# livesense-inc/fanlin-rs

Measured on AMD Instinct MI355X. Metric: images/sec whole-node (1080p→300×200 resize+encode); p50 per-image ms, higher is better.
Workload: dtype u8 (exact, as f16 subnormals) x the reference's f32 weights as three f16 terms -> f32 sums (vertical, v_mfma_f32_16x16x32_f16); 24-bit fixed-point intermediate (2^-14 steps, three i8 planes) x 24-bit fixed-point weights (2^-24 steps, three i8 digits), eight of the nine digit products -> exact i32 (h

## Files before the change

### fanlin-rs_amd/csrc/fl_jpeg.hip

```cpp
#include <hip/hip_runtime.h>
#include <stdint.h>

#include "fl_jpeg.h"
#include "fl_jpeg_tables.h"
#include "fl_pixel.h"
#include "fl_types.h"

namespace fl {

namespace {


constexpr int32_t F_0_298 = 2446, F_0_390 = 3196, F_0_541 = 4433, F_0_765 = 6270, F_0_899 = 7373, F_1_175 = 9633, F_1_501 = 12299,
                  F_1_847 = 15137, F_1_961 = 16069, F_2_053 = 16819, F_2_562 = 20995, F_3_072 = 25172;

struct Mat8 { int32_t a[8][8]; };

constexpr void fdct_linear(const int32_t in[8], int32_t out[8])
{
    int32_t t0 = in[0] + in[7], t1 = in[1] + in[6], t2 = in[2] + in[5], t3 = in[3] + in[4];
    const int32_t t10 = t0 + t3, t11 = t1 + t2;
    int32_t t12 = t0 - t3, t13 = t1 - t2;
    t0 = in[0] - in[7]; t1 = in[1] - in[6]; t2 = in[2] - in[5]; t3 = in[3] - in[4];
    out[0] = t10 + t11;
    out[4] = t10 - t11;
    int32_t z1 = (t12 + t13) * F_0_541;
    out[2] = z1 + t12 * F_0_765;
    out[6] = z1 - t13 * F_1_847;
    t12 = t0 + t2;
    t13 = t1 + t3;
    z1 = (t12 + t13) * F_1_175;
    t12 = t12 * (-F_0_390) + z1;
    t13 = t13 * (-F_1_961) + z1;
    z1 = (t0 + t3) * (-F_0_899);
    out[1] = t0 * F_1_501 + z1 + t12;
    out[7] = t3 * F_0_298 + z1 + t13;
    z1 = (t1 + t2) * (-F_2_562);
    out[3] = t1 * F_3_072 + z1 + t13;
    out[5] = t2 * F_2_053 + z1 + t12;
}

constexpr Mat8 make_fdct_matrix()
{
    Mat8 m{};
    for (int j = 0; j < 8; ++j) {
        int32_t e[8] = {0, 0, 0, 0, 0, 0, 0, 0}, o[8] = {0, 0, 0, 0, 0, 0, 0, 0};
        e[j] = 1;
        fdct_linear(e, o);
        for (int k = 0; k < 8; ++k) m.a[k][j] = o[k];
    }
    return m;
}

__constant__ Mat8 kFdct = make_fdct_matrix();

constexpr bool fdct_matrix_fits_i16()
{
    const Mat8 m = make_fdct_matrix();
    for (int k = 0; k < 8; ++k)
        for (int j = 0; j < 8; ++j)
            if (m.a[k][j] > 32767 || m.a[k][j] < -32768) return false;
    return true;
}
static_assert(fdct_matrix_fits_i16(), "the passes use v_dot2_i32_i16: matrix entries must be 16-bit");

typedef short i16x2 __attribute__((ext_vector_type(2)));
__device__ __forceinline__ i16x2 as_i16x2(uint32_t v) { return __builtin_bit_cast(i16x2, v); }
__device__ __forceinline__ uint32_t pack_i16(int32_t lo, int32_t hi) { return ((uint32_t)lo & 0xffffu) | ((uint32_t)hi << 16); }
__device__ __forceinline__ int32_t dot8_i16(const uint32_t m[4], const uint4 v)
{
    int32_t p = __builtin_amdgcn_sdot2(as_i16x2(m[0]), as_i16x2(v.x), 0, false);
    p = __builtin_amdgcn_sdot2(as_i16x2(m[1]), as_i16x2(v.y), p, false);
    p = __builtin_amdgcn_sdot2(as_i16x2(m[2]), as_i16x2(v.z), p, false);
    return __builtin_amdgcn_sdot2(as_i16x2(m[3]), as_i16x2(v.w), p, false);
}

struct NaturalOrder { uint8_t n[64]; };
constexpr NaturalOrder make_natural()
{
    NaturalOrder t{};
    for (int k = 0; k < 64; ++k) t.n[k] = kUnzigzag[k];
    return t;
}
__constant__ NaturalOrder kNatural = make_natural();

struct HuffLut { uint32_t e[256]; };

constexpr HuffLut make_lut(const HuffSpec &s)
{
    HuffLut t{};
    uint32_t code = 0;
    int k = 0;
    for (int l = 1; l <= 16; ++l) {
        for (int i = 0; i < s.len[l - 1]; ++i, ++k) t.e[s.val[k]] = ((uint32_t)l << 16) | code++;
        code <<= 1;
    }
    return t;
}

struct HuffAll { HuffLut ac[2], dc[2]; };
constexpr HuffAll make_all() { return HuffAll{{make_lut(kAcLuma), make_lut(kAcChroma)}, {make_lut(kDcLuma), make_lut(kDcChroma)}}; }
__constant__ HuffAll kHuff = make_all();


template <int N>
__device__ __forceinline__ uint32_t dpp_row_shr(uint32_t v)
{
    return (uint32_t)__builtin_amdgcn_update_dpp(0, (int)v, 0x110 + N, 0xf, 0xf, false);
}

__device__ __forceinline__ uint32_t wave_inclusive_scan(uint32_t v, uint32_t lane)
{
    (void)lane;
    v += dpp_row_shr<1>(v);
    v += dpp_row_shr<2>(v);
    v += dpp_row_shr<4>(v);
    v += dpp_row_shr<8>(v);
    v += (uint32_t)__builtin_amdgcn_update_dpp(0, (int)v, 0x142, 0xa, 0xf, false);
    v += (uint32_t)__builtin_amdgcn_update_dpp(0, (int)v, 0x143, 0xc, 0xf, false);
    return v;
}

__device__ __forceinline__ void wave_lds_sync()
{
    __builtin_amdgcn_fence(__ATOMIC_SEQ_CST, "wavefront");
    __builtin_amdgcn_wave_barrier();
}

constexpr uint32_t kPackThreads = 512;
constexpr uint32_t kPackWaves = kPackThreads / 64;

__device__ __forceinline__ uint32_t wg_exclusive_scan(uint32_t v, uint32_t *s_w, uint32_t *total)
{
    const uint32_t lane = threadIdx.x & 63u, wave = threadIdx.x >> 6;
    const uint32_t inc = wave_inclusive_scan(v, lane);
    __syncthreads();
    if (lane == 63u) s_w[wave] = inc;
    __syncthreads();
    uint32_t base = 0, sum = 0;
#pragma unroll
    for (uint32_t i = 0; i < kPackWaves; ++i) { const uint32_t t = s_w[i]; if (i < wave) base += t; sum += t; }
    *total = sum;
    return base + inc - v;
}

__device__ __forceinline__ uint32_t coef_size(int32_t v)
{
    const uint32_t mag = (uint32_t)(v < 0 ? -v : v);
    return mag ? 32u - (uint32_t)__clz(mag) : 0u;
}


#ifndef FL_JPEG_BPW
#define FL_JPEG_BPW 16
#define FL_JPEG_WPG 2
#define FL_JPEG_PREFETCH 3
#endif
constexpr uint32_t kBlocksPerWave = FL_JPEG_BPW;
constexpr uint32_t kWavesPerWg = FL_JPEG_WPG;
constexpr uint32_t kPrefetch = FL_JPEG_PREFETCH;
static_assert(kBlocksPerWave == 32u || kBlocksPerWave == 16u, "the coding phase's lane mapping");
constexpr uint32_t kJpegThreads = 64u * kWavesPerWg;
constexpr uint32_t kBlocksPerWg = kWavesPerWg * kBlocksPerWave;
constexpr uint32_t kUnitsPerWave = 3u * kBlocksPerWave;

static_assert(63u * (16u + 10u) <= kAcWordsPerUnit * 32u, "a unit's AC code must fit its acbits slot");

struct WaveLds {
    int16_t coef[kUnitsPerWave][64];
    uint64_t nz[kUnitsPerWave];
    __attribute__((aligned(16))) int16_t smp[3][64];
    __attribute__((aligned(16))) int16_t p1[3][64];
};

__device__ __forceinline__ void stage_ac_luts(uint32_t *s_ac)
{
    for (uint32_t i = threadIdx.x; i < 512u; i += kJpegThreads) s_ac[i] = kHuff.ac[i >> 8].e[i & 255u];
    __syncthreads();
}

template <bool kRgba>
__device__ __forceinline__ uint32_t block_pixel(const JpegJob &jb, uint32_t brow, uint32_t bcol, uint32_t r, uint32_t c)
{
    uint32_t px = bcol * 8u + c, py = brow * 8u + r;
    px = px < jb.w ? px : jb.w - 1u;
    py = py < jb.h ? py : jb.h - 1u;
    if constexpr (kRgba) return ((const __attribute__((address_space(1))) uint32_t *)jb.src)[(size_t)py * jb.w + px];
    uint32_t pr, pg, pb, pa;
    load_rgba(jb.src + ((size_t)py * jb.w + px) * jb.c, jb.c, pr, pg, pb, pa);
    return pr | (pg << 8) | (pb << 16);
}

__device__ __forceinline__ void dct_quant_block(const uint32_t (&smp)[3], uint32_t nat, uint32_t r, uint32_t c, const uint32_t (&m1)[4],
                                                const uint32_t (&m2)[4], uint4 k1, const uint32_t (&q)[3], const uint32_t (&magic)[3],
                                                WaveLds &w, int32_t (&qv)[3])
{
#pragma unroll
    for (int k = 0; k < 3; ++k) w.smp[k][nat] = (int16_t)smp[k];
    wave_lds_sync();
#pragma unroll
    for (int k = 0; k < 3; ++k) {
        const int32_t p = dot8_i16(m1, *reinterpret_cast<const uint4 *>(w.smp[k] + r * 8));
        const int32_t v1 = ((p << k1.x) + (int32_t)k1.y) >> 11;
        w.p1[k][c * 8 + r] = (int16_t)v1;
    }
    wave_lds_sync();
#pragma unroll
    for (int k = 0; k < 3; ++k) {
        const int32_t p2 = dot8_i16(m2, *reinterpret_cast<const uint4 *>(w.p1[k] + c * 8));
        const int32_t d = (p2 + (int32_t)k1.z) >> k1.w;
        const int32_t sg = d >> 31;
        const uint32_t an = (uint32_t)((d ^ sg) - sg) >> 3;
        const uint32_t rq = __umulhi(2u * an + q[k], magic[k]);
        qv[k] = ((int32_t)rq ^ sg) - sg;
    }
}

typedef __attribute__((address_space(1))) uint32_t global_u32;
typedef uint32_t u32x4 __attribute__((ext_vector_type(4)));
typedef __attribute__((address_space(1))) u32x4 global_u32x4;
static_assert(sizeof(JpegUnit) == sizeof(u32x4) && kUnitAcWords == 3u, "a unit's record is one 16-byte access");

struct UnitBits {
    uint64_t acc;
    uint32_t pend, total, wi;
    global_u32 *out;
    uint32_t w0, w1, w2;
    __device__ __forceinline__ void word(uint32_t v)
    {
        w0 = wi == 0u ? v : w0;
        w1 = wi == 1u ? v : w1;
        w2 = wi == 2u ? v : w2;
        if (wi >= kUnitAcWords) out[wi] = v;
        ++wi;
    }
    __device__ __forceinline__ void put(uint32_t code, uint32_t len)
    {
        acc = (acc << len) | code;
        pend += len;
        total += len;
        if (pend >= 32u) { pend -= 32u; word((uint32_t)(acc >> pend)); }
    }
};

template <bool kRgba>
__device__ __forceinline__ void transform_blocks(const JpegJob &jb, const uint32_t *__restrict__ arena, uint32_t first, uint32_t count,
                                                 uint32_t lane, WaveLds &w)
{
    const uint32_t nat = kNatural.n[lane], r = nat >> 3, c = nat & 7u;
    uint32_t m1[4], m2[4];
#pragma unroll
    for (int j = 0; j < 4; ++j) {
        m1[j] = pack_i16(kFdct.a[c][2 * j], kFdct.a[c][2 * j + 1]);
        m2[j] = pack_i16(kFdct.a[r][2 * j], kFdct.a[r][2 * j + 1]);
    }
    const uint8_t *qt = reinterpret_cast<const uint8_t *>(arena + jb.tab_off) + 624;
    const uint32_t *mg = reinterpret_cast<const uint32_t *>(qt + 128);
    const uint32_t q[3] = {qt[nat], qt[64 + nat], qt[64 + nat]};
    const uint32_t magic[3] = {mg[nat], mg[64 + nat], mg[64 + nat]};
    const uint4 k1 = {(c == 0u || c == 4u) ? 13u : 0u, c == 0u ? (uint32_t)(-(8 * 128) * 8192) : (c == 4u ? 0u : 1u << 10),
                      (r == 0u || r == 4u) ? 2u : 1u << 14, (r == 0u || r == 4u) ? 2u : 15u};
    uint32_t brow = first / jb.bx, bcol = first - brow * jb.bx;
    uint32_t ahead[kPrefetch];
#pragma unroll
    for (uint32_t j = 0; j < kPrefetch; ++j) {
        ahead[j] = block_pixel<kRgba>(jb, brow, bcol, r, c);
        if (++bcol == jb.bx) { bcol = 0; ++brow; }
    }
    for (uint32_t i = 0; i < count; ++i) {
        const uint32_t rgb = kRgba ? ahead[0] & 0xffffffu : ahead[0];
#pragma unroll
        for (uint32_t j = 0; j + 1u < kPrefetch; ++j) ahead[j] = ahead[j + 1u];
        ahead[kPrefetch - 1u] = block_pixel<kRgba>(jb, brow, bcol, r, c);
        if (++bcol == jb.bx) { bcol = 0; ++brow; }
        uint32_t smp[3];
        jfif_px(rgb, smp[0], smp[1], smp[2]);
        const bool flat = __ballot(rgb != (uint32_t)__builtin_amdgcn_readfirstlane((int)rgb)) == 0ull;
        if (flat) {
            if (lane == 0u) {
#pragma unroll
                for (int k = 0; k < 3; ++k) {
                    const int32_t d = 64 * ((int32_t)smp[k] - 128);
                    const int32_t sg = d >> 31;
                    const uint32_t an = (uint32_t)((d ^ sg) - sg) >> 3;
                    const uint32_t rq = __umulhi(2u * an + q[k], magic[k]);
                    w.coef[i * 3u + k][0] = (int16_t)(((int32_t)rq ^ sg) - sg);
                    w.nz[i * 3u + k] = 0ull;
                }
            }
            continue;
        }
        int32_t qv[3];
        dct_quant_block(smp, nat, r, c, m1, m2, k1, q, magic, w, qv);
#pragma unroll
        for (int k = 0; k < 3; ++k) {
            w.coef[i * 3u + k][lane] = (int16_t)qv[k];
            const uint64_t nz = __ballot(qv[k] != 0) & ~1ull;
            if (lane == 0u) w.nz[i * 3u + k] = nz;
        }
    }
}

__global__ __launch_bounds__(kJpegThreads) void jpeg_dct_quant_kernel(const JpegJob *__restrict__ jobs, const uint32_t *__restrict__ arena,
                                                                      uint32_t job_base)
{
    __shared__ WaveLds s_w[kWavesPerWg];
    __shared__ uint32_t s_ac[512];
    const JpegJob jb = jobs[job_base + blockIdx.y];
    const uint32_t wave = threadIdx.x >> 6, lane = threadIdx.x & 63u;
    const uint32_t nblocks = jb.bx * jb.by;
    if (blockIdx.x * kBlocksPerWg >= nblocks) return;
    stage_ac_luts(s_ac);
    const uint32_t first = blockIdx.x * kBlocksPerWg + wave * kBlocksPerWave;
    if (first >= nblocks) return;
    const uint32_t count = min(kBlocksPerWave, nblocks - first);
    WaveLds &w = s_w[wave];

    if (jb.c == 4u && (reinterpret_cast<uintptr_t>(jb.src) & 3u) == 0u) transform_blocks<true>(jb, arena, first, count, lane, w);
    else transform_blocks<false>(jb, arena, first, count, lane, w);
    wave_lds_sync();

    uint32_t b, u, u_end;
    bool chroma;
    if constexpr (kBlocksPerWave == 32u) {
        b = lane & 31u;
        chroma = lane >= 32u;
        u = b * 3u + (chroma ? 1u : 0u);
        u_end = b * 3u + (chroma ? 3u : 1u);
    } else {
        b = lane & 15u;
        chroma = lane >= 16u;
        u = b * 3u + (lane >> 4);
        u_end = lane >= 48u ? u : u + 1u;
    }
    if (b >= count) return;
    const uint32_t *tab = s_ac + (chroma ? 256u : 0u);
    const uint32_t eob = tab[0], zrl = tab[0xF0];
    for (; u < u_end; ++u) {
        const uint32_t unit = first * 3u + u;
        const int16_t *cf = w.coef[u];
        uint64_t m = w.nz[u];
        UnitBits ub{0ull, 0u, 0u, 0u, (global_u32 *)jb.acbits + (size_t)unit * kAcWordsPerUnit, 0u, 0u, 0u};
        uint32_t prev = 0;
        uint32_t pos = (uint32_t)__builtin_ctzll(m | (1ull << 63));
        int32_t v = cf[pos];
        while (m) {
            const uint32_t cpos = pos;
            const int32_t cv = v;
            m &= m - 1ull;
            pos = (uint32_t)__builtin_ctzll(m | (1ull << 63));
            v = cf[pos];
            uint32_t run = cpos - prev - 1u;
            prev = cpos;
            while (run > 15u) { ub.put(zrl & 0xffffu, zrl >> 16); run -= 16u; }
            const uint32_t mag = (uint32_t)(cv < 0 ? -cv : cv);
            const uint32_t size = 32u - (uint32_t)__clz(mag);
            const uint32_t value = (uint32_t)(cv + (cv >> 31)) & ((1u << size) - 1u);
            const uint32_t e = tab[(run << 4) | size];
            ub.put(((e & 0xffffu) << size) | value, (e >> 16) + size);
        }
        if (prev != 63u) ub.put(eob & 0xffffu, eob >> 16);
        if (ub.pend) ub.word((uint32_t)(ub.acc << (32u - ub.pend)));
        const u32x4 rec = {((uint32_t)(uint16_t)cf[0]) | (ub.total << 16), ub.w0, ub.w1, ub.w2};
        ((global_u32x4 *)jb.units)[unit] = rec;
    }
}


constexpr uint32_t kWinWords = 8192;

__device__ __forceinline__ void win_or(uint32_t *win, uint32_t wbase, uint64_t g, uint32_t val)
{
    const uint64_t W = g >> 5;
    const uint32_t sh = (uint32_t)g & 31u;
    const uint32_t hi = val >> sh, lo = sh ? val << (32u - sh) : 0u;
    if (hi && W >= wbase && W < (uint64_t)wbase + kWinWords) atomicOr(&win[W - wbase], hi);
    if (lo && W + 1 >= wbase && W + 1 < (uint64_t)wbase + kWinWords) atomicOr(&win[W + 1 - wbase], lo);
}

constexpr uint32_t kDcCodes = 12;

__device__ __forceinline__ uint32_t dc_code(const uint32_t *s_dc, uint32_t u, uint32_t meta, uint32_t prev_meta, uint32_t *len)
{
    const int32_t dc = (int16_t)(meta & 0xffffu), prev = (int16_t)(prev_meta & 0xffffu);
    const int32_t diff = dc - prev;
    const uint32_t size = coef_size(diff);
    const uint32_t value = (uint32_t)(diff < 0 ? diff - 1 : diff) & ((1u << size) - 1u);
    const uint32_t e = s_dc[((u % 3u) ? kDcCodes : 0u) + size];
    *len = (e >> 16) + size;
    return (((e & 0xffffu) << size) | value) << (32u - *len);
}

struct PackUnit { u32x4 rec; uint32_t prev; };
__device__ __forceinline__ PackUnit load_pack_unit(const JpegJob &jb, uint32_t u, uint32_t u_end)
{
    const global_u32x4 *recs = (const global_u32x4 *)jb.units;
    const uint32_t uc = min(u, u_end - 1u);
    PackUnit p;
    p.rec = recs[uc];
    p.prev = ((const global_u32 *)(recs + (max(uc, 3u) - 3u)))[0];
    return p;
}
__device__ __forceinline__ PackUnit take_pack_unit(PackUnit p, uint32_t u, uint32_t u_end)
{
    if (u >= u_end) p.rec = u32x4{0u, 0u, 0u, 0u};
    if (u < 3u || u >= u_end) p.prev = 0u;
    return p;
}

#ifndef FL_JPEG_PACK_DEPTH
#define FL_JPEG_PACK_DEPTH 1
#endif
constexpr uint32_t kPackDepth = FL_JPEG_PACK_DEPTH;

__global__ __launch_bounds__(kPackThreads) void jpeg_pack_kernel(const JpegJob *__restrict__ jobs, const uint32_t *__restrict__ arena,
                                                                 uint32_t job_base)
{
    __shared__ uint32_t s_win[kWinWords];
    __shared__ uint32_t s_w[kPackWaves], s_carry, s_lo, s_hi, s_dc[2u * kDcCodes];
    const JpegJob jb = jobs[job_base + blockIdx.x];
    const uint32_t tid = threadIdx.x;
    const uint32_t nunits = jb.bx * jb.by * 3u;
    constexpr uint32_t T = kPackThreads;

    PackUnit ahead[kPackDepth];
#pragma unroll
    for (uint32_t j = 0; j < kPackDepth; ++j) ahead[j] = load_pack_unit(jb, j * T + tid, nunits);
    for (uint32_t i = tid; i < kWinWords; i += T) s_win[i] = 0u;
    if (tid < 2u * kDcCodes) s_dc[tid] = kHuff.dc[tid / kDcCodes].e[tid % kDcCodes];
    if (tid == 0u) s_carry = 0u;
    __syncthreads();
    for (uint32_t base0 = 0; base0 < nunits; base0 += kPackDepth * T) {
#pragma unroll
        for (uint32_t j = 0; j < kPackDepth; ++j) {
            const uint32_t base = base0 + j * T;
            if (base >= nunits) break;
            const uint32_t u = base + tid;
            const PackUnit next = load_pack_unit(jb, u + kPackDepth * T, nunits);
            const PackUnit cur = take_pack_unit(ahead[j], u, nunits);
            ahead[j] = next;
            const uint32_t m = cur.rec.x;
            const uint32_t nw = ((m >> 16) + 31u) >> 5;
            uint32_t len = 0, dl = 0, dcw = 0;
            if (u < nunits) {
                dcw = dc_code(s_dc, u, m, cur.prev, &dl);
                len = dl + (m >> 16);
            }
            uint32_t chunk;
            const uint32_t ex = wg_exclusive_scan(len, s_w, &chunk);
            const uint32_t carry = s_carry;
            if (u < nunits) {
                const uint32_t off = carry + ex;
                ((global_u32 *)jb.unit_off)[u] = off;
                win_or(s_win, 0u, off, dcw);
                win_or(s_win, 0u, (uint64_t)off + dl, cur.rec.y);
                win_or(s_win, 0u, (uint64_t)off + dl + 32u, cur.rec.z);
                win_or(s_win, 0u, (uint64_t)off + dl + 64u, cur.rec.w);
                for (uint32_t w = kUnitAcWords; w < nw; ++w)
                    win_or(s_win, 0u, (uint64_t)off + dl + 32u * w, ((const global_u32 *)jb.acbits)[(size_t)u * kAcWordsPerUnit + w]);
            }
            __syncthreads();
            if (tid == 0u) s_carry = carry + chunk;
            __syncthreads();
        }
    }
    const uint32_t total_bits = s_carry;
    if (tid == 0u) jb.unit_off[nunits] = total_bits;
    __threadfence_block();
    __syncthreads();
    const uint32_t nbytes = (total_bits + 7u) >> 3, limit = jb.dst_cap;
    const uint8_t *hdr = reinterpret_cast<const uint8_t *>(arena + jb.tab_off);
    for (uint32_t i = tid; i < kJpegHeaderBytes; i += T) if (i < limit) jb.dst[i] = hdr[i];

    uint32_t ff_before = 0;
    for (uint32_t wbase = 0; wbase * 32ull < total_bits; wbase += kWinWords) {
        const uint64_t wb = (uint64_t)wbase * 32u, we = wb + (uint64_t)kWinWords * 32u;
        if (wbase != 0u) {
            for (uint32_t i = tid; i < kWinWords; i += T) s_win[i] = 0u;
            if (tid == 0u) {
                uint32_t lo = 0, hi = nunits;
                while (lo < hi) { const uint32_t mid = (lo + hi) >> 1; if (jb.unit_off[mid + 1u] > wb) hi = mid; else lo = mid + 1u; }
                s_lo = lo;
                uint32_t lo2 = lo, hi2 = nunits;
                while (lo2 < hi2) { const uint32_t mid = (lo2 + hi2) >> 1; if (jb.unit_off[mid] >= we) hi2 = mid; else lo2 = mid + 1u; }
                s_hi = lo2;
            }
        } else if (tid == 0u) { s_lo = 0u; s_hi = 0u; }
        __syncthreads();
        const uint32_t u_lo = s_lo, u_hi = s_hi;
        for (uint32_t ub = u_lo; ub < u_hi; ub += T / 2u) {
            const uint32_t u = ub + (tid >> 1), j = tid & 1u;
            if (u < u_hi) {
                const PackUnit p = take_pack_unit(load_pack_unit(jb, u, u_hi), u, u_hi);
                const uint32_t m = p.rec.x, off = jb.unit_off[u];
                uint32_t dl;
                const uint32_t dcw = dc_code(s_dc, u, m, p.prev, &dl);
                if (j == 0u) win_or(s_win, wbase, off, dcw);
                const uint32_t nw = ((m >> 16) + 31u) >> 5;
                win_or(s_win, wbase, (uint64_t)off + dl + 32u * j, j ? p.rec.z : p.rec.y);
                if (j == 0u) win_or(s_win, wbase, (uint64_t)off + dl + 64u, p.rec.w);
                for (uint32_t w = j ? 3u : 4u; w < nw; w += 2u)
                    win_or(s_win, wbase, (uint64_t)off + dl + 32u * w, ((const global_u32 *)jb.acbits)[(size_t)u * kAcWordsPerUnit + w]);
            }
        }
        __syncthreads();
        if (tid == 0u && (total_bits & 7u) && (total_bits >> 5) >= wbase && (total_bits >> 5) < wbase + kWinWords)
            s_win[(total_bits >> 5) - wbase] |= (0xFFu >> (total_bits & 7u)) << (24u - 8u * ((total_bits >> 3) & 3u));
        __syncthreads();
        const uint32_t win_bytes = (uint32_t)min((uint64_t)kWinWords * 4u, (uint64_t)nbytes - (uint64_t)wbase * 4u);
        if (tid == 0u) s_carry = 0u;
        __syncthreads();
        for (uint32_t base = 0; base < win_bytes; base += 4u * T) {
            const uint32_t i = base + tid * 4u;
            const uint32_t word = i < win_bytes ? s_win[i >> 2] : 0u;
            const uint32_t valid = i < win_bytes ? (win_bytes - i < 4u ? win_bytes - i : 4u) : 0u;
            uint32_t ff = 0;
#pragma unroll
            for (uint32_t k = 0; k < 4; ++k) ff += (k < valid && ((word >> (24u - 8u * k)) & 255u) == 255u) ? 1u : 0u;
            uint32_t chunk;
            const uint32_t ex = wg_exclusive_scan(ff, s_w, &chunk);
            const uint32_t carry = s_carry;
            uint64_t o = (uint64_t)kJpegHeaderBytes + (uint64_t)wbase * 4u + i + ff_before + carry + ex;
#pragma unroll
            for (uint32_t k = 0; k < 4; ++k) {
                if (k < valid) {
                    const uint32_t b = (word >> (24u - 8u * k)) & 255u;
                    if (o < limit) jb.dst[o] = (uint8_t)b;
                    ++o;
                    if (b == 255u) { if (o < limit) jb.dst[o] = 0u; ++o; }
                }
            }
            __syncthreads();
            if (tid == 0u) s_carry = carry + chunk;
            __syncthreads();
        }
        ff_before += s_carry;
        __syncthreads();
    }
    if (tid == 0u) {
        const uint64_t end = (uint64_t)kJpegHeaderBytes + nbytes + ff_before;
        if (end + 2u <= limit) {
            jb.dst[end] = 0xFF; jb.dst[end + 1u] = 0xD9;
            jb.result[1] = (uint32_t)(end + 2u);
        } else {
            jb.result[1] = 0u;
            atomicOr(&jb.result[0], FL_JPEG_RESULT_OVERFLOW);
        }
    }
}

}

hipError_t launch_jpeg_encode(const JpegJob *jobs, const uint32_t *arena, uint32_t job_base, uint32_t njobs, uint32_t max_blocks,
                              hipStream_t st)
{
    if (!njobs || !max_blocks) return hipSuccess;
    hipLaunchKernelGGL(jpeg_dct_quant_kernel, dim3((max_blocks + kBlocksPerWg - 1) / kBlocksPerWg, njobs), dim3(kJpegThreads), 0, st, jobs, arena, job_base);
    FL_LAUNCH_CHECK();
    hipLaunchKernelGGL(jpeg_pack_kernel, dim3(njobs), dim3(kPackThreads), 0, st, jobs, arena, job_base);
    FL_LAUNCH_CHECK();
    return hipSuccess;
}

}
```

Before: 558,700.

## Fold DCT rounding into dot seeds, use 32-bit pixel offsets, ring-buffer prefetch

Moves the pass-1 scale and bias into the DCT matrix and into the sdot2 accumulator seed, and folds the quantiser's shift and doubling into precomputed constants, which removes several ALU ops per coefficient. Adds a 32-bit offset path (v_mad_u32_u24) for pixel addressing when the image dimensions allow it, avoiding 64-bit address arithmetic. Replaces the shifting prefetch array with an indexed ring unrolled over kPrefetch and adds a sched_barrier. It also batches the lane-0 nz stores. The changed rounding constants must stay bit-exact, and the template instantiations double, which grows code size.

```diff
diff --git a/fanlin-rs_amd/csrc/fl_jpeg.hip b/fanlin-rs_amd/csrc/fl_jpeg.hip
--- a/fanlin-rs_amd/csrc/fl_jpeg.hip
+++ b/fanlin-rs_amd/csrc/fl_jpeg.hip
@@ -67,9 +67,9 @@
 typedef short i16x2 __attribute__((ext_vector_type(2)));
 __device__ __forceinline__ i16x2 as_i16x2(uint32_t v) { return __builtin_bit_cast(i16x2, v); }
 __device__ __forceinline__ uint32_t pack_i16(int32_t lo, int32_t hi) { return ((uint32_t)lo & 0xffffu) | ((uint32_t)hi << 16); }
-__device__ __forceinline__ int32_t dot8_i16(const uint32_t m[4], const uint4 v)
-{
-    int32_t p = __builtin_amdgcn_sdot2(as_i16x2(m[0]), as_i16x2(v.x), 0, false);
+__device__ __forceinline__ int32_t dot8_i16(const uint32_t m[4], const uint4 v, int32_t seed)
+{
+    int32_t p = __builtin_amdgcn_sdot2(as_i16x2(m[0]), as_i16x2(v.x), seed, false);
     p = __builtin_amdgcn_sdot2(as_i16x2(m[1]), as_i16x2(v.y), p, false);
     p = __builtin_amdgcn_sdot2(as_i16x2(m[2]), as_i16x2(v.z), p, false);
     return __builtin_amdgcn_sdot2(as_i16x2(m[3]), as_i16x2(v.w), p, false);
@@ -179,20 +179,39 @@
     __syncthreads();
 }
 
-template <bool kRgba>
+template <bool kRgba, bool kOff32>
 __device__ __forceinline__ uint32_t block_pixel(const JpegJob &jb, uint32_t brow, uint32_t bcol, uint32_t r, uint32_t c)
 {
     uint32_t px = bcol * 8u + c, py = brow * 8u + r;
     px = px < jb.w ? px : jb.w - 1u;
     py = py < jb.h ? py : jb.h - 1u;
+    if constexpr (kRgba && kOff32) {
+        uint32_t idx;
+        asm("v_mad_u32_u24 %0, %1, %2, %3" : "=v"(idx) : "v"(py), "s"(jb.w), "v"(px));
+        const uint32_t off = idx << 2;
+        return *(const __attribute__((address_space(1))) uint32_t *)((const __attribute__((address_space(1))) uint8_t *)jb.src + off);
+    }
     if constexpr (kRgba) return ((const __attribute__((address_space(1))) uint32_t *)jb.src)[(size_t)py * jb.w + px];
     uint32_t pr, pg, pb, pa;
-    load_rgba(jb.src + ((size_t)py * jb.w + px) * jb.c, jb.c, pr, pg, pb, pa);
+    if constexpr (kOff32) load_rgba(jb.src + ((py & 0xffffffu) * ((jb.w * jb.c) & 0xffffffu) + (px & 0xffffffu) * (jb.c & 0xffffffu)), jb.c, pr, pg, pb, pa);
+    else load_rgba(jb.src + ((size_t)py * jb.w + px) * jb.c, jb.c, pr, pg, pb, pa);
     return pr | (pg << 8) | (pb << 16);
 }
 
+__device__ __forceinline__ bool jpeg_offsets_fit_32bits(const JpegJob &jb)
+{
+    return (jb.w | jb.h) < 65536u && (uint64_t)(jb.w * jb.h) * jb.c <= (1ull << 32);
+}
+
+__device__ __forceinline__ int32_t quantise(int32_t d, uint32_t c8, uint32_t m8)
+{
+    const int32_t sg = d >> 31;
+    const uint32_t rq = __umulhi((uint32_t)((d ^ sg) - sg) + c8, m8);
+    return ((int32_t)rq ^ sg) - sg;
+}
+
 __device__ __forceinline__ void dct_quant_block(const uint32_t (&smp)[3], uint32_t nat, uint32_t r, uint32_t c, const uint32_t (&m1)[4],
-                                                const uint32_t (&m2)[4], uint4 k1, const uint32_t (&q)[3], const uint32_t (&magic)[3],
+                                                const uint32_t (&m2)[4], uint4 k1, const uint32_t (&c8)[3], const uint32_t (&m8)[3],
                                                 WaveLds &w, int32_t (&qv)[3])
 {
 #pragma unroll
@@ -200,19 +219,15 @@
     wave_lds_sync();
 #pragma unroll
     for (int k = 0; k < 3; ++k) {
-        const int32_t p = dot8_i16(m1, *reinterpret_cast<const uint4 *>(w.smp[k] + r * 8));
-        const int32_t v1 = ((p << k1.x) + (int32_t)k1.y) >> 11;
+        const int32_t p = dot8_i16(m1, *reinterpret_cast<const uint4 *>(w.smp[k] + r * 8), (int32_t)k1.y);
+        const int32_t v1 = p >> k1.x;
         w.p1[k][c * 8 + r] = (int16_t)v1;
     }
     wave_lds_sync();
 #pragma unroll
     for (int k = 0; k < 3; ++k) {
-        const int32_t p2 = dot8_i16(m2, *reinterpret_cast<const uint4 *>(w.p1[k] + c * 8));
-        const int32_t d = (p2 + (int32_t)k1.z) >> k1.w;
-        const int32_t sg = d >> 31;
-        const uint32_t an = (uint32_t)((d ^ sg) - sg) >> 3;
-        const uint32_t rq = __umulhi(2u * an + q[k], magic[k]);
-        qv[k] = ((int32_t)rq ^ sg) - sg;
+        const int32_t d = dot8_i16(m2, *reinterpret_cast<const uint4 *>(w.p1[k] + c * 8), (int32_t)k1.z) >> k1.w;
+        qv[k] = quantise(d, c8[k], m8[k]);
     }
 }
 
@@ -243,60 +258,69 @@
     }
 };
 
-template <bool kRgba>
+template <bool kRgba, bool kOff32>
 __device__ __forceinline__ void transform_blocks(const JpegJob &jb, const uint32_t *__restrict__ arena, uint32_t first, uint32_t count,
                                                  uint32_t lane, WaveLds &w)
 {
+    first = (uint32_t)__builtin_amdgcn_readfirstlane((int)first);
+    count = (uint32_t)__builtin_amdgcn_readfirstlane((int)count);
     const uint32_t nat = kNatural.n[lane], r = nat >> 3, c = nat & 7u;
     uint32_t m1[4], m2[4];
+    const int32_t pass1_scale = (c == 0u || c == 4u) ? 4 : 1;
 #pragma unroll
     for (int j = 0; j < 4; ++j) {
-        m1[j] = pack_i16(kFdct.a[c][2 * j], kFdct.a[c][2 * j + 1]);
+        m1[j] = pack_i16(pass1_scale * kFdct.a[c][2 * j], pass1_scale * kFdct.a[c][2 * j + 1]);
         m2[j] = pack_i16(kFdct.a[r][2 * j], kFdct.a[r][2 * j + 1]);
     }
     const uint8_t *qt = reinterpret_cast<const uint8_t *>(arena + jb.tab_off) + 624;
     const uint32_t *mg = reinterpret_cast<const uint32_t *>(qt + 128);
-    const uint32_t q[3] = {qt[nat], qt[64 + nat], qt[64 + nat]};
-    const uint32_t magic[3] = {mg[nat], mg[64 + nat], mg[64 + nat]};
-    const uint4 k1 = {(c == 0u || c == 4u) ? 13u : 0u, c == 0u ? (uint32_t)(-(8 * 128) * 8192) : (c == 4u ? 0u : 1u << 10),
+    const uint32_t c8[3] = {(qt[nat] & 0xfeu) << 2, (qt[64 + nat] & 0xfeu) << 2, (qt[64 + nat] & 0xfeu) << 2};
+    const uint32_t m8[3] = {(mg[nat] + 3u) >> 2, (mg[64 + nat] + 3u) >> 2, (mg[64 + nat] + 3u) >> 2};
+    const uint4 k1 = {(c == 0u || c == 4u) ? 0u : 11u, c == 0u ? (uint32_t)(-(8 * 128) * 4) : (c == 4u ? 0u : 1u << 10),
                       (r == 0u || r == 4u) ? 2u : 1u << 14, (r == 0u || r == 4u) ? 2u : 15u};
     uint32_t brow = first / jb.bx, bcol = first - brow * jb.bx;
     uint32_t ahead[kPrefetch];
 #pragma unroll
     for (uint32_t j = 0; j < kPrefetch; ++j) {
-        ahead[j] = block_pixel<kRgba>(jb, brow, bcol, r, c);
+        ahead[j] = block_pixel<kRgba, kOff32>(jb, brow, bcol, r, c);
         if (++bcol == jb.bx) { bcol = 0; ++brow; }
     }
-    for (uint32_t i = 0; i < count; ++i) {
-        const uint32_t rgb = kRgba ? ahead[0] & 0xffffffu : ahead[0];
-#pragma unroll
-        for (uint32_t j = 0; j + 1u < kPrefetch; ++j) ahead[j] = ahead[j + 1u];
-        ahead[kPrefetch - 1u] = block_pixel<kRgba>(jb, brow, bcol, r, c);
-        if (++bcol == jb.bx) { bcol = 0; ++brow; }
-        uint32_t smp[3];
-        jfif_px(rgb, smp[0], smp[1], smp[2]);
+    auto one_block = [&](uint32_t i, uint32_t rgb, const uint32_t (&smp)[3]) __attribute__((always_inline)) {
         const bool flat = __ballot(rgb != (uint32_t)__builtin_amdgcn_readfirstlane((int)rgb)) == 0ull;
         if (flat) {
             if (lane == 0u) {
 #pragma unroll
                 for (int k = 0; k < 3; ++k) {
-                    const int32_t d = 64 * ((int32_t)smp[k] - 128);
-                    const int32_t sg = d >> 31;
-                    const uint32_t an = (uint32_t)((d ^ sg) - sg) >> 3;
-                    const uint32_t rq = __umulhi(2u * an + q[k], magic[k]);
-                    w.coef[i * 3u + k][0] = (int16_t)(((int32_t)rq ^ sg) - sg);
+                    w.coef[i * 3u + k][0] = (int16_t)quantise(64 * ((int32_t)smp[k] - 128), c8[k], m8[k]);
                     w.nz[i * 3u + k] = 0ull;
                 }
             }
-            continue;
+            return;
         }
         int32_t qv[3];
-        dct_quant_block(smp, nat, r, c, m1, m2, k1, q, magic, w, qv);
+        dct_quant_block(smp, nat, r, c, m1, m2, k1, c8, m8, w, qv);
+        uint64_t nz[3];
 #pragma unroll
         for (int k = 0; k < 3; ++k) {
             w.coef[i * 3u + k][lane] = (int16_t)qv[k];
-            const uint64_t nz = __ballot(qv[k] != 0) & ~1ull;
-            if (lane == 0u) w.nz[i * 3u + k] = nz;
+            nz[k] = __ballot(qv[k] != 0) & ~1ull;
+        }
+        if (lane == 0u) {
+#pragma unroll
+            for (int k = 0; k < 3; ++k) w.nz[i * 3u + k] = nz[k];
+        }
+    };
+    for (uint32_t i0 = 0; i0 < count; i0 += kPrefetch) {
+#pragma unroll
+        for (uint32_t j = 0; j < kPrefetch; ++j) {
+            if (i0 + j >= count) break;
+            const uint32_t rgb = kRgba ? ahead[j] & 0xffffffu : ahead[j];
+            uint32_t smp[3];
+            jfif_px(rgb, smp[0], smp[1], smp[2]);
+            __builtin_amdgcn_sched_barrier(0);
+            ahead[j] = block_pixel<kRgba, kOff32>(jb, brow, bcol, r, c);
+            if (++bcol == jb.bx) { bcol = 0; ++brow; }
+            one_block(i0 + j, rgb, smp);
         }
     }
 }
@@ -316,8 +340,14 @@
     const uint32_t count = min(kBlocksPerWave, nblocks - first);
     WaveLds &w = s_w[wave];
 
-    if (jb.c == 4u && (reinterpret_cast<uintptr_t>(jb.src) & 3u) == 0u) transform_blocks<true>(jb, arena, first, count, lane, w);
-    else transform_blocks<false>(jb, arena, first, count, lane, w);
+    const bool rgba = jb.c == 4u && (reinterpret_cast<uintptr_t>(jb.src) & 3u) == 0u;
+    if (jpeg_offsets_fit_32bits(jb)) {
+        if (rgba) transform_blocks<true, true>(jb, arena, first, count, lane, w);
+        else transform_blocks<false, true>(jb, arena, first, count, lane, w);
+    } else {
+        if (rgba) transform_blocks<true, false>(jb, arena, first, count, lane, w);
+        else transform_blocks<false, false>(jb, arena, first, count, lane, w);
+    }
     wave_lds_sync();
 
     uint32_t b, u, u_end;
```

Measured after the change: 563,300, median of 5. About the same (+0.8%).
